# sheepTnT/Stage-IndexOrganized

Measured on AMD Instinct MI355X. Metric: YCSB ops/sec at 1/2/4/8 GPU + achieved HBM GB/s vs peak; CPU ref ops/sec, higher is better.
Workload: dtype u64; 1 GPU; YCSB-C 100M rows uint64 keys, zipf 0.9, batched point-lookup on 1×MI355X; traversal=device, rows_per_gpu=100000000, rows_total=100000000, batch_per_gpu=16777216, key_bytes=8, payload_bytes=1000, leaf_bytes=65536, parallelism=single GPU

## Files before the change

stage-indexorganized_amd/csrc/kernel_api.hpp:

```cpp
#pragma once
#include <hip/hip_runtime_api.h>

#include <cstdint>

#include "stage_core.hpp"

namespace stage {

struct alignas(16) stage_probe_out_dev {
    uint32_t w[8];
};

struct alignas(8) ImageDescDev {
    uint64_t key_le;
    uint64_t arg;
    uint32_t kind;
    uint32_t mode;
};

constexpr int kProbeFormWave = 0, kProbeFormLane = 1;
struct ProbeTuning {
    int group = 8;
    int max_blocks = 0;
    int store = 1;
    int status_bytes = 32;
    int form = kProbeFormLane;
};
constexpr int kProbeRows = 16;

hipError_t launch_resolve(const DevTable &t, const uint64_t *keys, const uint16_t *lens, uint64_t n, int le_child,
                          uint32_t *out, hipStream_t s);
hipError_t launch_probe(const DevTable &t, const uint64_t *keys, const uint16_t *lens, const uint32_t *rids,
                        const uint32_t *leaf_in, uint64_t n, stage_probe_out_dev *out, uint8_t *recs, hipStream_t s,
                        const ProbeTuning &tune, const uint64_t *d_n = nullptr, uint64_t shape_n = 0);
hipError_t launch_probe_window(const DevTable &t, const uint64_t *keys, const uint16_t *lens, const uint32_t *rids,
                               const uint32_t *leaf_in, uint64_t n, uint32_t row_off, uint32_t len,
                               stage_probe_out_dev *out, uint8_t *win, hipStream_t s, const ProbeTuning &tune);
bool probe_missed_supported(const DevTable &t);
hipError_t launch_probe_missed(const DevTable &t, const uint64_t *keys, uint64_t n, stage_probe_out_dev *out,
                               hipStream_t s, const ProbeTuning &tune, const uint64_t *d_n, uint64_t shape_n,
                               const uint32_t *mrids, uint32_t mnq, int32_t *missed);
struct alignas(8) FanRange {
    uint32_t lo, hi;
};
constexpr int kFanDests = 64;
struct FanDest {
    uint32_t nseg;
    uint32_t end[kFanDests];
    stage_probe_out_dev *out[kFanDests];
    uint8_t *recs[kFanDests];
};
bool probe_fanout_supported(const DevTable &t);
hipError_t launch_probe_fanout(const DevTable &t, const uint64_t *keys, const uint32_t *rids, uint64_t n,
                               const FanRange *fan, const uint32_t *flist, stage_probe_out_dev *out, uint8_t *recs,
                               hipStream_t s, const ProbeTuning &tune, const FanDest *dest = nullptr);
struct ScanTuning {
    int max_blocks = 0;
};

hipError_t launch_scan(const DevTable &t, const uint64_t *keys, const uint16_t *lens, uint64_t n, uint32_t scan_size,
                       uint32_t *counts, uint8_t *recs, hipStream_t s, const ScanTuning &tune,
                       const uint32_t *rids = nullptr, uint8_t *row_status = nullptr);
hipError_t launch_scan_window(const DevTable &t, const uint64_t *keys, const uint16_t *lens, uint64_t n,
                              uint32_t scan_size, uint32_t row_off, uint32_t len, uint32_t key_pad, uint32_t *counts,
                              uint8_t *win, uint8_t *row_keys, hipStream_t s, const ScanTuning &tune,
                              const uint32_t *rids = nullptr, uint8_t *row_status = nullptr);
struct TableScanOut {
    uint64_t max_records;
    uint64_t *count;
    uint64_t *leaf_offsets;
    uint8_t *recs;
    uint8_t *win;
    uint8_t *row_keys;
    uint64_t *row_meta;
    uint8_t *row_status;
};
uint64_t table_scan_scratch_bytes(uint64_t nl);
hipError_t launch_table_scan(const DevTable &t, uint32_t leaf0, uint32_t nl, bool snapshot, uint32_t rid,
                             uint32_t row_off, uint32_t len, uint32_t key_pad, const TableScanOut &o, uint8_t *scratch,
                             hipStream_t s, const ScanTuning &tune);
hipError_t launch_scan_pair(const DevTable &t0, const uint64_t *k0, uint32_t sz0, uint32_t *c0, uint8_t *r0,
                            const DevTable &t1, const uint64_t *k1, uint32_t sz1, uint32_t *c1, uint8_t *r1,
                            hipStream_t s);
bool scan_pair_supported(const DevTable &t0, uint32_t sz0, const DevTable &t1, uint32_t sz1);
hipError_t launch_scan_first(const DevTable &t, const uint64_t *keys, uint64_t n, uint32_t scan_size,
                             const uint32_t *rids, uint32_t words, uint32_t *img_out, uint8_t *st_out, hipStream_t s,
                             const ScanTuning &tune);
struct alignas(16) ReaderReq {
    uint64_t key;
    uint32_t rid;
    uint32_t tag;
};
struct ReaderRing {
    const ReaderReq *req;
    uint32_t *done;
    stage_probe_out_dev *out;
    uint8_t *rows;
    const uint32_t *stop;
    uint64_t *pos;
    uint32_t slots;
    uint32_t waves;
    uint64_t life_ticks;
    uint32_t *ident;
};
hipError_t launch_resident_reader(const DevTable &t, const ReaderRing &g, hipStream_t s);
hipError_t launch_revisit(const DevTable &t, const stage_probe_out_dev *base, uint64_t n, const uint32_t *rids,
                          uint32_t nq, const uint32_t *perm, stage_probe_out_dev *out, hipStream_t s,
                          const uint64_t *d_n = nullptr);
hipError_t launch_revisit_segments(const DevTable &t, const stage_probe_out_dev *base, uint64_t n,
                                   const uint64_t *seg_off, const uint32_t *seg_cnt, uint32_t nseg,
                                   const uint32_t *rids, uint32_t nq, stage_probe_out_dev *last, int32_t *missed,
                                   hipStream_t s, const uint64_t *d_n = nullptr, const uint64_t *d_nseg = nullptr);
hipError_t launch_for_update(const DevTable &t, const uint8_t *fu, const uint32_t *rids, uint64_t n,
                             stage_probe_out_dev *out, uint8_t *recs, hipStream_t s);
hipError_t launch_ident(const DevTable &t, const stage_probe_out_dev *out, uint64_t n, uint32_t *ident, hipStream_t s);
hipError_t launch_murmur(const void *keys, uint32_t key_len, uint32_t key_stride, uint64_t seed, uint64_t n,
                         uint64_t *out, hipStream_t s);
hipError_t launch_fill(uint8_t *heap, uint32_t stride, uint32_t payload_size, uint32_t row_bytes,
                       const ImageDescDev *descs, const uint8_t *arena, uint64_t first, uint64_t count,
                       uint64_t ident_rowid0, uint32_t ident_key_width, int ident_mode, hipStream_t s);
hipError_t launch_patch(uint8_t *head, uint64_t *okey, SlotInfo *slot, uint32_t head_bytes, uint32_t cap, uint32_t kw,
                        const uint32_t *head_leaf, const void *head_src, uint64_t nhead, const uint64_t *slot_idx,
                        const SlotInfo *slot_src, const uint64_t *words, uint64_t nslot, hipStream_t s);

}
```

stage-indexorganized_amd/csrc/probe.hip:

```cpp
#include <algorithm>

#include "kernel_api.hpp"
#include "launch_util.hpp"
#include "row_store.hpp"
#include "tree_search.hpp"

namespace stage {

template <int KW>
__global__ __launch_bounds__(256) void resolve_kernel(DevTable t, const uint64_t *__restrict__ keys,
                                                      const uint16_t *__restrict__ lens, uint64_t n, int le_child,
                                                      uint32_t *__restrict__ out) {
    uint64_t i = (uint64_t)blockIdx.x * blockDim.x + threadIdx.x;
    if (i >= n) return;
    uint32_t len = t.key_width ? t.key_width : (lens ? lens[i] : 8u);
    uint64_t ok[KW];
    load_okey<KW>(keys, i, true, len, ok);
    out[i] = t.key_width ? resolve_leaf<false, KW>(t, ok, len, le_child != 0)
                         : resolve_leaf<true, 1>(t, ok, len, le_child != 0);
}


template <bool VARLEN, int SPL, int G, int POL = 1, int ST = 32, bool FAN = false, bool DEST = false>
__global__ __launch_bounds__(256) void probe_kernel(DevTable t, const uint64_t *__restrict__ keys,
// ... 488 lines not shown
    const uint32_t out_chunks = t.stride >> 4;
    const uint32_t len = t.key_width;
    for (uint64_t base = wave * CH; base < n; base += nwaves * CH) {
        const uint64_t i = base + lane;
        const bool valid = lane < (uint32_t)CH && i < n;
        const uint32_t rid = rids ? (valid ? rids[i] : 0u) : 0xFFFFFFFEu;
        uint64_t ok[KW];
        load_okey<KW>(keys, i, valid, len, ok);
        uint32_t leaf = 0;
        if (valid) leaf = leaf_in ? leaf_in[i] : resolve_leaf<false, KW>(t, ok, len, true);
        if (leaf > t.nseps) leaf = t.nseps;
        const uint32_t fx_mine = key_fp_words(ok, KW);
        const int cnt = (int)((n - base) < CH ? (n - base) : CH);
        constexpr int PD = SPL <= 4 ? 4 : 1;
        uint32_t pf[PD][SPL];
#pragma unroll
        for (int d = 0; d < PD; ++d) {
            if (d < cnt) {
                const uint8_t *h = t.head + (uint64_t)rl32(leaf, d) * t.head_bytes;
#pragma unroll
                for (int s = 0; s < SPL; ++s) pf[d][s] = h[s * 64 + lane];
            }
        }
        uint32_t my_nc = 0;
        for (int j0 = 0; j0 < cnt; j0 += PD) {
#pragma unroll
            for (int u = 0; u < PD; ++u) {
                const int j = j0 + u;
                if (j >= cnt) break;
                uint32_t fpb[SPL];
#pragma unroll
                for (int s = 0; s < SPL; ++s) fpb[s] = pf[u][s];
                if (j + PD < cnt) {
                    const uint8_t *h = t.head + (uint64_t)rl32(leaf, j + PD) * t.head_bytes;
#pragma unroll
                    for (int s = 0; s < SPL; ++s) pf[u][s] = h[s * 64 + lane];
                }
                const uint32_t fx = rl32(fx_mine, j);
                uint32_t nc = 0;
#pragma unroll
                for (int s = 0; s < SPL; ++s) {
                    const bool c = fpb[s] == fx;
                    const uint64_t cm = ballot(c);
                    const uint32_t r = nc + count_below(cm);
                    if (c && r < (uint32_t)kProbeCand) s_cand[wv][j][r] = (uint16_t)(s * 64 + lane);
                    nc += (uint32_t)__builtin_popcountll(cm);
                }
                if (lane == (uint32_t)j) my_nc = nc;
            }
        }
        __builtin_amdgcn_fence(__ATOMIC_RELEASE, "wavefront");
        __builtin_amdgcn_wave_barrier();
        __builtin_amdgcn_fence(__ATOMIC_ACQUIRE, "wavefront");
        int slot = -1;
        uint64_t m = 0;
        uint32_t nx = 0, im = 0;
        if (valid) {
            const uint64_t lb = (uint64_t)leaf * t.cap;
            if (my_nc <= (uint32_t)kProbeCand) {
                for (uint32_t c = 0; c < my_nc; ++c)
                    if (confirm_slot<KW>(t, leaf, lb, s_cand[wv][lane][c], ok, slot, m, nx, im)) break;
            } else {
                const uint8_t *h = t.head + (uint64_t)leaf * t.head_bytes;
                for (uint32_t sl = 0; sl < t.cap; ++sl)
                    if (h[sl] == fx_mine && confirm_slot<KW>(t, leaf, lb, sl, ok, slot, m, nx, im)) break;
            }
        }
        ProbeRes r;
        visibility(t, slot, m, nx, im, rid, r);
        store_chunk(t, lane, base, cnt, valid, leaf, r, out, recs, out_chunks);
        __builtin_amdgcn_wave_barrier();
    }
}

template <int KW>
__device__ __forceinline__ uint32_t coop_lower_bound(const DevTable &t, const uint64_t *ok, uint32_t lane,
                                                     uint64_t *s_x, uint32_t *s_node) {
#pragma unroll
    for (int j = 0; j < KW; ++j) s_x[lane * KW + j] = ok[j];
    uint32_t node = 0;
    for (int lvl = (int)t.levels - 1; lvl >= 0; --lvl) {
        const uint32_t f = lvl > 0 ? (uint32_t)kTreeFanout : (uint32_t)kLeafFanout;
        const uint32_t sh = lvl > 0 ? 4u : 3u, kpr = 64u >> sh;
        const uint32_t rounds = 64u / kpr;
        s_node[lane] = node;
        __builtin_amdgcn_wave_barrier();
        const uint64_t lbase = t.level_off[lvl];
        const uint32_t e = lane & (f - 1), kq = lane >> sh;
        const uint32_t my_round = lane / kpr, my_team = lane % kpr;
        uint64_t ball = 0;
        constexpr int kBatch = 8;
#pragma unroll
        for (int r0 = 0; r0 < 16; r0 += kBatch) {
            if ((uint32_t)r0 >= rounds) break;
            uint64_t w[kBatch][KW];
#pragma unroll
            for (int r = 0; r < kBatch; ++r) {
                const uint32_t kk = (uint32_t)(r0 + r) * kpr + kq;
                const uint64_t ent = lbase + (uint64_t)s_node[kk] * f + e;
#pragma unroll
                for (int j = 0; j < KW; ++j) w[r][j] = t.tree[ent * KW + j];
            }
#pragma unroll
            for (int r = 0; r < kBatch; ++r) {
                const uint32_t kk = (uint32_t)(r0 + r) * kpr + kq;
                uint64_t x[KW];
#pragma unroll
                for (int j = 0; j < KW; ++j) x[j] = s_x[kk * KW + j];
                const uint64_t b = __builtin_amdgcn_ballot_w64(kw_lt<KW>(w[r], x));
                ball = (uint32_t)(r0 + r) == my_round ? b : ball;
            }
        }
        const uint32_t cnt = (uint32_t)__builtin_popcountll((ball >> (my_team * f)) & ((1ull << f) - 1));
        node = node * f + cnt;
        __builtin_amdgcn_wave_barrier();
    }
    return node < t.nseps ? node : t.nseps;
}

template <int SPL, int KW, bool MISS = false>
__global__ __launch_bounds__(256) void probe_lane_kernel(DevTable t, const uint64_t *__restrict__ keys,
                                                         const uint32_t *__restrict__ rids,
                                                         const uint32_t *__restrict__ leaf_in, uint64_t n,
                                                         stage_probe_out_dev *__restrict__ out,
                                                         uint8_t *__restrict__ recs, const uint64_t *__restrict__ dn,
                                                         const uint32_t *__restrict__ mrids = nullptr,
                                                         uint32_t mnq = 0, int32_t *__restrict__ missed = nullptr) {
    static_assert(SPL <= 4, "head of at most 256 slots in registers");
    __shared__ uint64_t s_x[4][64 * KW];
    __shared__ uint32_t s_node[4][64];
    if (dn) n = *dn < n ? *dn : n;
    const uint32_t lane = lane_id(), wv = uni32(threadIdx.x >> 6);
    const uint64_t wave = (uint64_t)blockIdx.x * (blockDim.x >> 6) + wv;
    const uint64_t nwaves = (uint64_t)gridDim.x * (blockDim.x >> 6);
    const uint32_t out_chunks = t.stride >> 4;
    const uint32_t len = t.key_width;
    for (uint64_t base = wave * 64; base < n; base += nwaves * 64) {
        const uint64_t i = base + lane;
        const bool valid = i < n;
        const uint32_t rid = rids ? (valid ? rids[i] : 0u) : 0xFFFFFFFEu;
        uint64_t ok[KW];
        load_okey<KW>(keys, i, valid, len, ok);
        uint32_t leaf = 0;
        if (leaf_in) leaf = valid ? leaf_in[i] : 0u;
        else leaf = coop_lower_bound<KW>(t, ok, lane, s_x[wv], s_node[wv]);
        if (!valid) leaf = 0;
        if (leaf > t.nseps) leaf = t.nseps;
        const uint32_t rep = (key_fp_words(ok, KW) & 0xFFu) * 0x01010101u;
        u32x4 hv[SPL * 4];
        const u32x4 *hp = reinterpret_cast<const u32x4 *>(t.head + (uint64_t)leaf * t.head_bytes);
#pragma unroll
        for (int q = 0; q < SPL * 4; ++q) hv[q] = valid ? hp[q] : u32x4{0, 0, 0, 0};
        uint32_t c0 = 0, c1 = 0, c2 = 0, nc = 0;
#pragma unroll
        for (int q = 0; q < SPL * 4; ++q) {
            const uint32_t wq[4] = {hv[q].x, hv[q].y, hv[q].z, hv[q].w};
#pragma unroll
            for (int e = 0; e < 4; ++e) {
                const uint32_t w = wq[e] ^ rep;
                uint32_t zm = ~(((w & 0x7F7F7F7Fu) + 0x7F7F7F7Fu) | w) & 0x80808080u;
                while (zm) {
                    const uint32_t sl = (uint32_t)(q * 16 + e * 4) + ((uint32_t)__builtin_ctz(zm) >> 3);
                    c0 = nc == 0 ? sl : c0;
                    c1 = nc == 1 ? sl : c1;
                    c2 = nc == 2 ? sl : c2;
                    ++nc;
                    zm &= zm - 1;
                }
            }
        }
        if (!valid) nc = 0;
        int slot = -1;
        uint64_t m = 0;
        uint32_t nx = 0, im = 0;
        const uint64_t lb = (uint64_t)leaf * t.cap;
        auto confirm = [&](uint32_t sl) { return confirm_slot<KW>(t, leaf, lb, sl, ok, slot, m, nx, im); };
        if (nc > 0) confirm(c0);
        if (slot < 0 && nc > 1) confirm(c1);
        if (slot < 0 && nc > 2) confirm(c2);
        if (slot < 0 && nc > 3) {
            const uint8_t *h = t.head + (uint64_t)leaf * t.head_bytes;
            const uint8_t fx = (uint8_t)rep;
            for (uint32_t sl = c2 + 1; sl < t.cap; ++sl)
                if (h[sl] == fx && confirm(sl)) break;
        }
        ProbeRes r;
        visibility(t, slot, m, nx, im, rid, r);
        if (MISS && valid)
            for (uint32_t q = 0; q < mnq; ++q) {
                ProbeRes rq;
                visibility(t, slot, m, nx, im, mrids[q], rq);
                if (rq.status != ST_LATEST && rq.status != ST_COPY && rq.status != ST_OLD) atomicOr(missed + q, 1);
            }
        store_chunk(t, lane, base, (int)((n - base) < 64 ? (n - base) : 64), valid, leaf, r, out, recs, out_chunks);
    }
}

template <int SPL, int R, int ST>
__global__ __launch_bounds__(256) void probe_rows_kernel(DevTable t, const uint64_t *__restrict__ keys,
                                                         const uint32_t *__restrict__ rids,
                                                         const uint32_t *__restrict__ leaf_in, uint64_t n,
                                                         stage_probe_out_dev *__restrict__ out,
                                                         uint8_t *__restrict__ recs) {
    static_assert(SPL <= 2, "probe_kernel's leaves: 64 or 128 slots");
    const uint32_t lane = lane_id();
    const uint64_t wave = (uint64_t)blockIdx.x * (blockDim.x >> 6) + uni32(threadIdx.x >> 6);
    const uint64_t nwaves = (uint64_t)gridDim.x * (blockDim.x >> 6);
    const uint32_t out_chunks = t.stride >> 4;
    const uint32_t len = t.key_width;
    for (uint64_t base = wave * 64; base < n; base += nwaves * 64) {
        const uint64_t i = base + lane;
        const bool valid = i < n;
        const uint32_t rid = rids ? (valid ? rids[i] : 0u) : 0xFFFFFFFEu;
        uint64_t ok;
        load_okey<1>(keys, i, valid, len, &ok);
        uint32_t leaf = 0;
        if (valid) leaf = leaf_in ? leaf_in[i] : resolve_leaf<false, 1>(t, &ok, len, true);
        if (leaf > t.nseps) leaf = t.nseps;
        const uint32_t rep = (key_fp_words(&ok, 1) & 0xFFu) * 0x01010101u;
        u32x4 hv[SPL * 4];
        const u32x4 *hp = reinterpret_cast<const u32x4 *>(t.head + (uint64_t)leaf * t.head_bytes);
#pragma unroll
        for (int q = 0; q < SPL * 4; ++q) hv[q] = valid ? hp[q] : u32x4{0, 0, 0, 0};
        uint32_t c0 = 0, c1 = 0, c2 = 0, nc = 0;
#pragma unroll
        for (int q = 0; q < SPL * 4; ++q) {
            const uint32_t wq[4] = {hv[q].x, hv[q].y, hv[q].z, hv[q].w};
#pragma unroll
            for (int e = 0; e < 4; ++e) {
                const uint32_t w = wq[e] ^ rep;
                uint32_t zm = ~(((w & 0x7F7F7F7Fu) + 0x7F7F7F7Fu) | w) & 0x80808080u;
                while (zm) {
                    const uint32_t sl = (uint32_t)(q * 16 + e * 4) + ((uint32_t)__builtin_ctz(zm) >> 3);
                    c0 = nc == 0 ? sl : c0;
                    c1 = nc == 1 ? sl : c1;
                    c2 = nc == 2 ? sl : c2;
                    ++nc;
                    zm &= zm - 1;
                }
            }
        }
        if (!valid) nc = 0;
        int slot = -1;
        uint64_t m = 0;
        uint32_t nx = 0, im = 0;
        const uint64_t lb = (uint64_t)leaf * t.cap;
        auto confirm = [&](uint32_t sl) { return confirm_slot<1>(t, leaf, lb, sl, &ok, slot, m, nx, im); };
        if (nc > 0) confirm(c0);
        if (slot < 0 && nc > 1) confirm(c1);
        if (slot < 0 && nc > 2) confirm(c2);
        if (slot < 0 && nc > 3) {
            const uint8_t *h = t.head + (uint64_t)leaf * t.head_bytes;
            const uint8_t fx = (uint8_t)rep;
            for (uint32_t sl = c2 + 1; sl < t.cap; ++sl)
                if (h[sl] == fx && confirm(sl)) break;
        }
        ProbeRes r;
        if (slot >= 0 && !meta_inserting(m) && rid >= meta_cstamp(m) && (nx & kNextKindMask) != kNextCopy) {
            r.status = ST_LATEST;
            r.flags = 0;
            r.hops = 0;
            r.slot = (uint32_t)slot;
            r.meta_hi = (uint32_t)(m >> 32);
            r.cstamp = rid;
            r.rec_cstamp = meta_cstamp(m);
            r.copy_sstamp = kMaxCid;
            r.image = im;
        } else {
            visibility(t, slot, m, nx, im, rid, r);
        }
        if (valid) {
            u32x4 a, b;
            pack_out(leaf, r, a, b);
            if constexpr (ST == 16) {
                st16<1>(u32x4{a.x, a.w, b.y, b.x}, reinterpret_cast<uint8_t *>(out) + base * 16u, lane * 16u);
            } else {
                uint8_t *ob = reinterpret_cast<uint8_t *>(out + base);
                st16<1>(a, ob, lane * 32u);
                st16<1>(b, ob, lane * 32u + 16u);
            }
        }
        if (!recs) continue;
        const int cnt = (int)((n - base) < 64 ? (n - base) : 64);
        for (int j0 = 0; j0 < cnt; j0 += R) {
            for (uint32_t k0 = 0; k0 < out_chunks; k0 += 64) {
                const uint32_t c = k0 + lane;
                u32x4 v[R];
#pragma unroll
                for (int g = 0; g < R; ++g) {
                    const uint32_t img = rl32(r.image, j0 + g < cnt ? j0 + g : cnt - 1);
                    v[g] = u32x4{0, 0, 0, 0};
                    if (c < out_chunks && img != 0xFFFFFFFFu) v[g] = heap_chunk(t, img, c);
                }
#pragma unroll
                for (int g = 0; g < R; ++g) {
                    const int j = j0 + g;
                    if (j < cnt && c < out_chunks) st16<1>(v[g], recs + (base + j) * (uint64_t)t.stride, c * 16u);
                }
            }
        }
    }
}


hipError_t launch_resolve(const DevTable &t, const uint64_t *keys, const uint16_t *lens, uint64_t n, int le_child,
                          uint32_t *out, hipStream_t s) {
    if (n == 0) return hipSuccess;
    const unsigned b = (unsigned)((n + 255) / 256);
    with_key_words(t, [&](auto KW) { resolve_kernel<KW()><<<b, 256, 0, s>>>(t, keys, lens, n, le_child, out); });
    return hipGetLastError();
}

constexpr uint64_t kSmallBelow = 16384;

hipError_t launch_probe(const DevTable &t, const uint64_t *keys, const uint16_t *lens, const uint32_t *rids,
                        const uint32_t *leaf_in, uint64_t n, stage_probe_out_dev *out, uint8_t *recs, hipStream_t s,
                        const ProbeTuning &tune, const uint64_t *d_n, uint64_t shape_n) {
    if (n == 0) return hipSuccess;
    if (d_n) {
        if (!(t.key_words > 1 || (t.key_width != 0 && t.cap > 128))) return hipErrorInvalidValue;
    }
    const int mb = max_blocks(tune);
    const int blocks = grid_for((n + 63) / 64, 4, mb);
    const bool var = t.key_width == 0;
    if (t.key_words > 1 || (!var && t.cap > 128)) {
        const uint64_t sn = d_n && shape_n ? std::min(shape_n, n) : n;
        const bool small = (sn + 63) / 64 < (uint64_t)kSmallBelow;
        const bool tiny = (sn + 15) / 16 < (uint64_t)kSmallBelow / 4;
        with_geometry(t, [&](auto S, auto KW) {
            if constexpr (S() <= 4) {
                probe_lane_kernel<S(), KW()><<<grid_for((sn + 63) / 64, 4, mb), 256, 0, s>>>(t, keys, rids, leaf_in, n,
                                                                                             out, recs, d_n);
            } else if (tiny) {
                probe_split_kernel<S(), KW(), 4><<<grid_for((sn + 3) / 4, 4, mb), 256, 0, s>>>(t, keys, rids, leaf_in, n,
                                                                                               out, recs, d_n);
            } else if (small) {
                probe_split_kernel<S(), KW(), 16><<<grid_for((sn + 15) / 16, 4, mb), 256, 0, s>>>(t, keys, rids, leaf_in,
                                                                                                  n, out, recs, d_n);
            } else {
                probe_split_kernel<S(), KW(), 64><<<blocks, 256, 0, s>>>(t, keys, rids, leaf_in, n, out, recs, d_n);
            }
        });
        return hipGetLastError();
    }
    if (!var && tune.form == kProbeFormLane && tune.group == 8 && tune.store == 1 &&
        (tune.status_bytes != 16 || t.cap == 64)) {
        auto launch_rows = [&](auto kernel) { kernel<<<blocks, 256, 0, s>>>(t, keys, rids, leaf_in, n, out, recs); };
        if (tune.status_bytes == 16) launch_rows(probe_rows_kernel<1, kProbeRows, 16>);
        else if (t.cap == 64) launch_rows(probe_rows_kernel<1, kProbeRows, 32>);
        else launch_rows(probe_rows_kernel<2, kProbeRows, 32>);
        return hipGetLastError();
    }
    auto launch = [&](auto kernel) {
        kernel<<<blocks, 256, 0, s>>>(t, keys, lens, rids, leaf_in, n, out, recs, nullptr, nullptr, nullptr);
    };
    if (tune.status_bytes == 16) {
        if (var || t.cap != 64 || tune.group != 8 || tune.store != 1) return hipErrorInvalidValue;
        launch(probe_kernel<false, 1, 8, 1, 16>);
        return hipGetLastError();
    }
    if (t.cap == 64) {
        if (var) launch(probe_kernel<true, 1, 4>);
        else if (tune.group == 1) launch(probe_kernel<false, 1, 1>);
        else if (tune.group == 2) launch(probe_kernel<false, 1, 2>);
        else if (tune.group == 4) launch(probe_kernel<false, 1, 4>);
        else if (tune.store == 0) launch(probe_kernel<false, 1, 8, 0>);
        else if (tune.store == 2) launch(probe_kernel<false, 1, 8, 2>);
        else launch(probe_kernel<false, 1, 8>);
    } else {
        if (var) launch(probe_kernel<true, 2, 4>);
        else launch(probe_kernel<false, 2, 4>);
    }
    return hipGetLastError();
}

hipError_t launch_probe_window(const DevTable &t, const uint64_t *keys, const uint16_t *lens, const uint32_t *rids,
                               const uint32_t *leaf_in, uint64_t n, uint32_t row_off, uint32_t len,
                               stage_probe_out_dev *out, uint8_t *win, hipStream_t s, const ProbeTuning &tune) {
    if (len == 0 || (uint64_t)row_off + len > t.hstride || (n && !win)) return hipErrorInvalidValue;
    if (n == 0) return hipSuccess;
    const WindowArgs w{row_off, len, (len + 15u) >> 4, win};
    const int mb = max_blocks(tune);
    const int blocks = grid_for((n + 63) / 64, 4, mb);
    const bool var = t.key_width == 0;
    if (t.key_words > 1 || (!var && t.cap > 128)) {
        ProbeTuning full = tune;
        full.status_bytes = 32;
        const hipError_t e = launch_probe(t, keys, lens, rids, leaf_in, n, out, nullptr, s, full);
        if (e != hipSuccess) return e;
        window_gather_kernel<<<blocks, 256, 0, s>>>(t, out, n, w);
        return hipGetLastError();
    }
    if (tune.status_bytes == 16 && (var || t.cap != 64)) return hipErrorInvalidValue;
    hipError_t e = hipErrorInvalidValue;
    with_slot_groups(t, [&](auto S) {
        if constexpr (S() <= 2) {
            auto launch = [&](auto kernel) {
                kernel<<<blocks, 256, 0, s>>>(t, keys, lens, rids, leaf_in, n, out, w);
                e = hipGetLastError();
            };
            if (var) {
                launch(probe_window_kernel<true, S(), 4, 32>);
            } else if constexpr (S() == 1) {
                if (tune.status_bytes == 16) launch(probe_window_kernel<false, 1, 8, 16>);
                else launch(probe_window_kernel<false, 1, 8, 32>);
            } else {
                launch(probe_window_kernel<false, 2, 4, 32>);
            }
        }
    });
    return e;
}

hipError_t launch_probe_missed(const DevTable &t, const uint64_t *keys, uint64_t n, stage_probe_out_dev *out,
                               hipStream_t s, const ProbeTuning &tune, const uint64_t *d_n, uint64_t shape_n,
                               const uint32_t *mrids, uint32_t mnq, int32_t *missed) {
    if (!probe_missed_supported(t)) return hipErrorInvalidValue;
    if (n == 0) return hipSuccess;
    const uint64_t sn = d_n && shape_n ? std::min(shape_n, n) : n;
    const int blocks = grid_for((sn + 63) / 64, 4, max_blocks(tune));
    with_geometry(t, [&](auto S, auto KW) {
        if constexpr (S() <= 4)
            probe_lane_kernel<S(), KW(), true><<<blocks, 256, 0, s>>>(t, keys, nullptr, nullptr, n, out, nullptr, d_n,
                                                                      mrids, mnq, missed);
    });
    return hipGetLastError();
}

bool probe_missed_supported(const DevTable &t) {
    const bool wide = t.key_words > 1 || (t.key_width != 0 && t.cap > 128);
    return wide && t.key_width != 0 && t.cap <= 256 && (t.cap == 64 || t.cap == 128 || t.cap == 256);
}

hipError_t launch_probe_fanout(const DevTable &t, const uint64_t *keys, const uint32_t *rids, uint64_t n,
                               const FanRange *fan, const uint32_t *flist, stage_probe_out_dev *out, uint8_t *recs,
                               hipStream_t s, const ProbeTuning &tune, const FanDest *dest) {
    if (!probe_fanout_supported(t)) return hipErrorInvalidValue;
    if (n == 0) return hipSuccess;
    if ((!recs && !dest) || (!fan && !flist)) return hipErrorInvalidValue;
    const int blocks = grid_for((n + 63) / 64, 4, max_blocks(tune));
    if (dest)
        probe_kernel<false, 1, 4, 1, 32, true, true><<<blocks, 256, 0, s>>>(t, keys, nullptr, rids, nullptr, n, out,
                                                                            recs, fan, flist, dest);
    else
        probe_kernel<false, 1, 8, 1, 32, true><<<blocks, 256, 0, s>>>(t, keys, nullptr, rids, nullptr, n, out, recs,
                                                                      fan, flist);
    return hipGetLastError();
}

bool probe_fanout_supported(const DevTable &t) {
    return t.key_width != 0 && t.key_words == 1 && t.cap == 64 && t.stride <= 1024;
}

__global__ __launch_bounds__(256) void revisit_kernel(DevTable t, const stage_probe_out_dev *__restrict__ base,
                                                      uint64_t n, const uint32_t *__restrict__ rids, uint32_t nq,
                                                      const uint32_t *__restrict__ perm,
                                                      stage_probe_out_dev *__restrict__ out,
                                                      const uint64_t *__restrict__ dn) {
    if (dn) n = *dn < n ? *dn : n;
    const uint64_t g = (uint64_t)blockIdx.x * blockDim.x + threadIdx.x;
    if (g >= n * nq) return;
    const uint64_t i = g % n, q = g / n;
    const u32x4 *bp = reinterpret_cast<const u32x4 *>(base + i);
    u32x4 a = bp[0], b = bp[1];
    revisit_one(t, rids[q], a, b);
    u32x4 *op = reinterpret_cast<u32x4 *>(out + q * n + (perm ? perm[i] : i));
    op[0] = a;
    op[1] = b;
}

constexpr uint32_t kRevisitQ = 16;
__global__ __launch_bounds__(256) void revisit_missed_kernel(DevTable t, const stage_probe_out_dev *__restrict__ base,
                                                             uint64_t n, const uint32_t *__restrict__ rids, uint32_t nq,
                                                             int32_t *__restrict__ missed, const uint64_t *__restrict__ dn) {
    if (dn) n = *dn < n ? *dn : n;
    const uint64_t g = (uint64_t)blockIdx.x * blockDim.x + threadIdx.x;
    if (g >= n * ((nq + kRevisitQ - 1) / kRevisitQ)) return;
    const uint64_t i = g % n;
    const uint32_t q0 = (uint32_t)(g / n) * kRevisitQ, q1 = q0 + kRevisitQ < nq ? q0 + kRevisitQ : nq;
    const u32x4 *bp = reinterpret_cast<const u32x4 *>(base + i);
    const u32x4 a0 = bp[0];
    const uint32_t slot = a0.z & 0xFFFF, leaf = a0.y;
    const bool redo = (a0.x & 0xFF) != ST_NOT_FOUND && slot < t.cap && leaf < t.nleaves;
    SlotInfo si = {};
    if (redo) si = t.slot[(uint64_t)leaf * t.cap + slot];
    for (uint32_t q = q0; q < q1; ++q) {
        uint32_t st = a0.x & 0xFF;
        if (redo) {
            ProbeRes r;
            visibility(t, (int)slot, si.meta, si.next, si.image, rids[q], r);
            st = r.status;
        }
        if (st != ST_LATEST && st != ST_COPY && st != ST_OLD) atomicOr(missed + q, 1);
    }
}

__global__ __launch_bounds__(256) void revisit_last_kernel(DevTable t, const stage_probe_out_dev *__restrict__ base,
                                                           const uint64_t *__restrict__ seg_off,
                                                           const uint32_t *__restrict__ seg_cnt, uint32_t nseg,
                                                           const uint32_t *__restrict__ rids, uint32_t nq,
                                                           stage_probe_out_dev *__restrict__ last,
                                                           const uint64_t *__restrict__ dseg) {
    if (dseg) nseg = *dseg < nseg ? (uint32_t)*dseg : nseg;
    const uint64_t g = (uint64_t)blockIdx.x * blockDim.x + threadIdx.x;
    if (g >= (uint64_t)nseg * nq) return;
    const uint32_t k = (uint32_t)(g % nseg), q = (uint32_t)(g / nseg);
    const uint32_t c = seg_cnt[k];
    if (c == 0) return;
    const u32x4 *bp = reinterpret_cast<const u32x4 *>(base + seg_off[k] + c - 1);
    u32x4 a = bp[0], b = bp[1];
    revisit_one(t, rids[q], a, b);
    u32x4 *op = reinterpret_cast<u32x4 *>(last + g);
    op[0] = a;
    op[1] = b;
}

hipError_t launch_revisit_segments(const DevTable &t, const stage_probe_out_dev *base, uint64_t n,
                                   const uint64_t *seg_off, const uint32_t *seg_cnt, uint32_t nseg,
                                   const uint32_t *rids, uint32_t nq, stage_probe_out_dev *last, int32_t *missed,
                                   hipStream_t s, const uint64_t *d_n, const uint64_t *d_nseg) {
    if (nq == 0) return hipSuccess;
    const uint64_t tm = n * ((nq + kRevisitQ - 1) / kRevisitQ), tl = (uint64_t)nseg * nq;
    if (tm) revisit_missed_kernel<<<(unsigned)((tm + 255) / 256), 256, 0, s>>>(t, base, n, rids, nq, missed, d_n);
    if (tl)
        revisit_last_kernel<<<(unsigned)((tl + 255) / 256), 256, 0, s>>>(t, base, seg_off, seg_cnt, nseg, rids, nq, last,
                                                                         d_nseg);
    return hipGetLastError();
}

hipError_t launch_revisit(const DevTable &t, const stage_probe_out_dev *base, uint64_t n, const uint32_t *rids,
                          uint32_t nq, const uint32_t *perm, stage_probe_out_dev *out, hipStream_t s,
                          const uint64_t *d_n) {
    if (n == 0 || nq == 0) return hipSuccess;
    revisit_kernel<<<(unsigned)((n * nq + 255) / 256), 256, 0, s>>>(t, base, n, rids, nq, perm, out, d_n);
    return hipGetLastError();
}

__global__ __launch_bounds__(256) void ident_kernel(DevTable t, const stage_probe_out_dev *__restrict__ out, uint64_t n,
                                                    uint32_t *__restrict__ ident) {
    const uint64_t i = (uint64_t)blockIdx.x * blockDim.x + threadIdx.x;
    if (i >= n) return;
    const u32x4 a = reinterpret_cast<const u32x4 *>(out + i)[0];
    const uint32_t status = a.x & 0xFF, leaf = a.y, slot = a.z & 0xFFFF;
    uint32_t loc = 0, next = 0;
    if (status != ST_NOT_FOUND && slot < t.cap && leaf < t.nleaves) {
        const u32x4 w1 = reinterpret_cast<const u32x4 *>(t.slot + (uint64_t)leaf * t.cap + slot)[1];
        next = w1.x;
        loc = w1.z;
    }
    reinterpret_cast<uint2 *>(ident)[i] = make_uint2(loc, next);
}

__global__ __launch_bounds__(256) void for_update_kernel(DevTable t, const uint8_t *__restrict__ fu,
                                                         const uint32_t *__restrict__ rids, uint64_t n,
                                                         stage_probe_out_dev *__restrict__ out, uint8_t *__restrict__ recs) {
    const uint32_t lane = lane_id();
    const uint64_t base = ((uint64_t)blockIdx.x * (blockDim.x >> 6) + uni32(threadIdx.x >> 6)) * 64;
    const uint64_t i = base + lane;
    uint64_t todo = ballot(i < n && fu[i] != 0);
    const uint32_t chunks = t.stride >> 4;
    while (todo) {
        const int j = __builtin_ctzll(todo);
        todo &= todo - 1;
        const uint64_t p = base + (uint64_t)j;
        const u32x4 *op = reinterpret_cast<const u32x4 *>(out + p);
        u32x4 a = op[0], b = op[1];
        const uint32_t rid = rids ? rids[p] : 0xFFFFFFFEu;
        const uint32_t slot = a.z & 0xFFFF, leaf = a.y;
        uint32_t image = 0xFFFFFFFFu;
        if (slot < t.cap && leaf < t.nleaves) {
            const SlotInfo si = t.slot[(uint64_t)leaf * t.cap + slot];
            ProbeRes r;
            visibility<true>(t, (int)slot, si.meta, si.next, si.image, rid, r);
            pack_out(leaf, r, a, b);
            image = r.image;
        } else {
            a.x |= 2u << 8;
        }
        if (lane < 2) reinterpret_cast<u32x4 *>(out + p)[lane] = lane == 0 ? a : b;
        if (recs) {
            for (uint32_t c = lane; c < chunks; c += 64) {
                u32x4 v = u32x4{0, 0, 0, 0};
                if (image != 0xFFFFFFFFu) v = heap_chunk(t, image, c);
                reinterpret_cast<u32x4 *>(recs + p * (uint64_t)t.stride)[c] = v;
            }
        }
    }
}

hipError_t launch_for_update(const DevTable &t, const uint8_t *fu, const uint32_t *rids, uint64_t n,
                             stage_probe_out_dev *out, uint8_t *recs, hipStream_t s) {
    if (n == 0) return hipSuccess;
    for_update_kernel<<<(unsigned)((n + 255) / 256), 256, 0, s>>>(t, fu, rids, n, out, recs);
    return hipGetLastError();
}

hipError_t launch_ident(const DevTable &t, const stage_probe_out_dev *out, uint64_t n, uint32_t *ident, hipStream_t s) {
    if (n == 0) return hipSuccess;
    ident_kernel<<<(unsigned)((n + 255) / 256), 256, 0, s>>>(t, out, n, ident);
    return hipGetLastError();
}

hipError_t launch_resident_reader(const DevTable &t, const ReaderRing &g, hipStream_t s) {
    if (t.key_words != 1 || g.waves == 0 || g.slots % (64 * g.waves)) return hipErrorInvalidValue;
    const dim3 grid(g.waves), block(64);
    if (t.key_width == 0 && t.cap > 128) return hipErrorInvalidValue;
    with_slot_groups(t, [&](auto S) {
        if (t.key_width != 0) resident_reader_kernel<false, S()><<<grid, block, 0, s>>>(t, g);
        else if constexpr (S() <= 2) resident_reader_kernel<true, S()><<<grid, block, 0, s>>>(t, g);
    });
    return hipGetLastError();
}

}
```

Measured before the change: 2.767 billion ops/s.

## Add lane-per-key fanout probe kernel with batched row gathers

Adds a new fanout probe kernel in which each lane resolves its own key, does a fingerprint SIMD match over the leaf head, and confirms candidates. The wave then cooperatively gathers R record rows at a time and scatters them to all fan-out destinations, with nontemporal stores for the status words. The default tuning dispatches to this kernel instead of the older wave-per-key probe_kernel. The aim is to cut per-key serialisation and increase memory-level parallelism in the row gather. The cost is more registers (R row vectors held per lane) and a fallback serial scan when a leaf has more than three fingerprint hits.

New measurement: 2.767 billion ops/s, median of 2. No clear change (-0.0%).

```diff
diff --git a/stage-indexorganized_amd/csrc/kernel_api.hpp b/stage-indexorganized_amd/csrc/kernel_api.hpp
--- a/stage-indexorganized_amd/csrc/kernel_api.hpp
+++ b/stage-indexorganized_amd/csrc/kernel_api.hpp
@@ -27,6 +27,10 @@
     int form = kProbeFormLane;
 };
 constexpr int kProbeRows = 16;
+#ifndef STAGE_FAN_ROWS
+#define STAGE_FAN_ROWS 16
+#endif
+constexpr int kFanRows = STAGE_FAN_ROWS;
 
 hipError_t launch_resolve(const DevTable &t, const uint64_t *keys, const uint16_t *lens, uint64_t n, int le_child,
                           uint32_t *out, hipStream_t s);
diff --git a/stage-indexorganized_amd/csrc/probe.hip b/stage-indexorganized_amd/csrc/probe.hip
--- a/stage-indexorganized_amd/csrc/probe.hip
+++ b/stage-indexorganized_amd/csrc/probe.hip
@@ -814,6 +814,150 @@
     }
 }
 
+template <bool DEST, int R>
+__global__ __launch_bounds__(256) void probe_fan_rows_kernel(DevTable t, const uint64_t *__restrict__ keys,
+                                                             const uint32_t *__restrict__ rids, uint64_t n,
+                                                             stage_probe_out_dev *__restrict__ out,
+                                                             uint8_t *__restrict__ recs,
+                                                             const FanRange *__restrict__ fan,
+                                                             const uint32_t *__restrict__ flist,
+                                                             const FanDest *__restrict__ dest) {
+    const uint32_t lane = lane_id();
+    __shared__ uint32_t s_dend[DEST ? kFanDests : 1];
+    __shared__ stage_probe_out_dev *s_dout[DEST ? kFanDests : 1];
+    __shared__ uint8_t *s_drec[DEST ? kFanDests : 1];
+    uint32_t nseg = 0;
+    if constexpr (DEST) {
+        nseg = dest->nseg;
+        for (uint32_t g = threadIdx.x; g < nseg; g += blockDim.x)
+            s_dend[g] = dest->end[g], s_dout[g] = dest->out[g], s_drec[g] = dest->recs[g];
+        __syncthreads();
+    }
+    const uint64_t wave = (uint64_t)blockIdx.x * (blockDim.x >> 6) + uni32(threadIdx.x >> 6);
+    const uint64_t nwaves = (uint64_t)gridDim.x * (blockDim.x >> 6);
+    const uint32_t out_chunks = t.stride >> 4;
+    const uint32_t len = t.key_width;
+    for (uint64_t base = wave * 64; base < n; base += nwaves * 64) {
+        const uint64_t i = base + lane;
+        const bool valid = i < n;
+        const uint32_t rid = rids ? (valid ? rids[i] : 0u) : 0xFFFFFFFEu;
+        FanRange my_fan = FanRange{0u, 0u};
+        if (valid) my_fan = fan ? fan[i] : FanRange{(uint32_t)i, (uint32_t)i + 1u};
+        uint64_t my_o = (uint64_t)out, my_r = (uint64_t)recs;
+        if constexpr (DEST) {
+            uint32_t sg = 0;
+            for (uint32_t g = 0; g + 1 < nseg; ++g) sg += i >= s_dend[g] ? 1u : 0u;
+            my_o = (uint64_t)s_dout[sg];
+            my_r = (uint64_t)s_drec[sg];
+        }
+        uint64_t ok;
+        load_okey<1>(keys, i, valid, len, &ok);
+        uint32_t leaf = 0;
+        if (valid) leaf = resolve_leaf<false, 1>(t, &ok, len, true);
+        if (leaf > t.nseps) leaf = t.nseps;
+        const uint32_t rep = (key_fp_words(&ok, 1) & 0xFFu) * 0x01010101u;
+        u32x4 hv[4];
+        const u32x4 *hp = reinterpret_cast<const u32x4 *>(t.head + (uint64_t)leaf * t.head_bytes);
+#pragma unroll
+        for (int q = 0; q < 4; ++q) hv[q] = valid ? hp[q] : u32x4{0, 0, 0, 0};
+        uint32_t c0 = 0, c1 = 0, c2 = 0, nc = 0;
+#pragma unroll
+        for (int q = 0; q < 4; ++q) {
+            const uint32_t wq[4] = {hv[q].x, hv[q].y, hv[q].z, hv[q].w};
+#pragma unroll
+            for (int e = 0; e < 4; ++e) {
+                const uint32_t w = wq[e] ^ rep;
+                uint32_t zm = ~(((w & 0x7F7F7F7Fu) + 0x7F7F7F7Fu) | w) & 0x80808080u;
+                while (zm) {
+                    const uint32_t sl = (uint32_t)(q * 16 + e * 4) + ((uint32_t)__builtin_ctz(zm) >> 3);
+                    c0 = nc == 0 ? sl : c0;
+                    c1 = nc == 1 ? sl : c1;
+                    c2 = nc == 2 ? sl : c2;
+                    ++nc;
+                    zm &= zm - 1;
+                }
+            }
+        }
+        if (!valid) nc = 0;
+        int slot = -1;
+        uint64_t m = 0;
+        uint32_t nx = 0, im = 0;
+        const uint64_t lb = (uint64_t)leaf * t.cap;
+        auto confirm = [&](uint32_t sl) { return confirm_slot<1>(t, leaf, lb, sl, &ok, slot, m, nx, im); };
+        if (nc > 0) confirm(c0);
+        if (slot < 0 && nc > 1) confirm(c1);
+        if (slot < 0 && nc > 2) confirm(c2);
+        if (slot < 0 && nc > 3) {
+            const uint8_t *h = t.head + (uint64_t)leaf * t.head_bytes;
+            const uint8_t fx = (uint8_t)rep;
+            for (uint32_t sl = c2 + 1; sl < t.cap; ++sl)
+                if (h[sl] == fx && confirm(sl)) break;
+        }
+        ProbeRes r;
+        if (slot >= 0 && !meta_inserting(m) && rid >= meta_cstamp(m) && (nx & kNextKindMask) != kNextCopy) {
+            r.status = ST_LATEST;
+            r.flags = 0;
+            r.hops = 0;
+            r.slot = (uint32_t)slot;
+            r.meta_hi = (uint32_t)(m >> 32);
+            r.cstamp = rid;
+            r.rec_cstamp = meta_cstamp(m);
+            r.copy_sstamp = kMaxCid;
+            r.image = im;
+        } else {
+            visibility(t, slot, m, nx, im, rid, r);
+        }
+        u32x4 my_a, my_b;
+        pack_out(leaf, r, my_a, my_b);
+        const int cnt = (int)((n - base) < 64 ? (n - base) : 64);
+        for (int j0 = 0; j0 < cnt; j0 += R) {
+            u32x4 v[R];
+            uint32_t mine0[R];
+#pragma unroll
+            for (int g = 0; g < R; ++g) {
+                const int j = j0 + g < cnt ? j0 + g : cnt - 1;
+                const uint32_t img = rl32(r.image, j);
+                v[g] = u32x4{0, 0, 0, 0};
+                if (lane < out_chunks && img != 0xFFFFFFFFu) v[g] = heap_chunk(t, img, lane);
+                const uint32_t lo = rl32(my_fan.lo, j), hi = rl32(my_fan.hi, j);
+                const uint32_t kk = lo + lane;
+                mine0[g] = j0 + g < cnt && kk < hi ? (flist ? flist[kk] : kk) : 0u;
+            }
+#pragma unroll
+            for (int g = 0; g < R; ++g) {
+                const int j = j0 + g;
+                if (j >= cnt) break;
+                const u32x4 a = u32x4{rl32(my_a.x, j), rl32(my_a.y, j), rl32(my_a.z, j), rl32(my_a.w, j)};
+                const u32x4 b = u32x4{rl32(my_b.x, j), rl32(my_b.y, j), rl32(my_b.z, j), rl32(my_b.w, j)};
+                const uint32_t lo = rl32(my_fan.lo, j), hi = rl32(my_fan.hi, j);
+                stage_probe_out_dev *o_j = out;
+                uint8_t *r_j = recs;
+                if constexpr (DEST) {
+                    o_j = reinterpret_cast<stage_probe_out_dev *>(rl64(my_o, j));
+                    r_j = reinterpret_cast<uint8_t *>(rl64(my_r, j));
+                }
+                auto store = [&](uint32_t mine, uint32_t kn) {
+                    for (uint32_t k = 0; k < kn; ++k) {
+                        const uint64_t pos = rl32(mine, (int)k);
+                        if (lane < out_chunks) st16<1>(v[g], r_j + pos * (uint64_t)t.stride, lane * 16u);
+                    }
+                    const u32x4 half = lane & 1u ? b : a;
+                    for (uint32_t h = 0; h < kn; h += 32) {
+                        const uint32_t kp = h + (lane >> 1);
+                        const uint32_t p = (uint32_t)__shfl((int)mine, (int)kp);
+                        if (kp < kn) __builtin_nontemporal_store(half, reinterpret_cast<u32x4 *>(o_j + p) + (lane & 1u));
+                    }
+                };
+                store(mine0[g], hi - lo < 64u ? hi - lo : 64u);
+                for (uint32_t k0 = lo + 64; k0 < hi; k0 += 64) {
+                    const uint32_t kk = k0 + lane;
+                    store(kk < hi ? (flist ? flist[kk] : kk) : 0u, hi - k0 < 64u ? hi - k0 : 64u);
+                }
+            }
+        }
+    }
+}
+
 
 hipError_t launch_resolve(const DevTable &t, const uint64_t *keys, const uint16_t *lens, uint64_t n, int le_child,
                           uint32_t *out, hipStream_t s) {
@@ -951,6 +1095,14 @@
     if (n == 0) return hipSuccess;
     if ((!recs && !dest) || (!fan && !flist)) return hipErrorInvalidValue;
     const int blocks = grid_for((n + 63) / 64, 4, max_blocks(tune));
+    if (tune.form == kProbeFormLane && tune.group == 8 && tune.store == 1) {
+        if (dest)
+            probe_fan_rows_kernel<true, kFanRows><<<blocks, 256, 0, s>>>(t, keys, rids, n, out, recs, fan, flist, dest);
+        else
+            probe_fan_rows_kernel<false, kFanRows><<<blocks, 256, 0, s>>>(t, keys, rids, n, out, recs, fan, flist,
+                                                                         nullptr);
+        return hipGetLastError();
+    }
     if (dest)
         probe_kernel<false, 1, 4, 1, 32, true, true><<<blocks, 256, 0, s>>>(t, keys, nullptr, rids, nullptr, n, out,
                                                                             recs, fan, flist, dest);
```
